# SeanNaren/deepspeech.pytorch

Measured on AMD Instinct MI355X. Metric: audio-seconds/sec (train step), higher is better.
Workload: dtype bf16

## Files before the change

deepspeech/pytorch_amd/_lib.py:

```python
import ctypes as C
import os

HERE = os.path.dirname(os.path.abspath(__file__))
LIB_PATH = os.path.join(HERE, "libds2hip.so")

F32, BF16 = 0, 1
CELL_GRU, CELL_LSTM, CELL_RNN_TANH = 0, 1, 2

_vp, _i, _l, _f, _ll = C.c_void_p, C.c_int, C.c_long, C.c_float, C.c_longlong

SIGNATURES = {
    "ds2_version": (_i, []),
    "ds2_error_string": (C.c_char_p, [_i]),
    "ds2_gemm_nt": (_i, [_i, _vp, _vp, _vp, _vp, _i, _i, _i, _l, _l, _l, _i, _i, _l, _l, _l, _l, _i, _vp]),
    "ds2_gemm_nt_coresident": (_i, [_i, _vp, _vp, _vp, _vp, _i, _i, _i, _l, _l, _l, _i, _i, _l, _l, _l, _l, _i, _vp]),
    "ds2_gemm_nt_rows2": (_i, [_i, _vp, _vp, _i, _vp, _vp, _i, _i, _i, _l, _l, _l, _i, _i, _i, _vp]),
    "ds2_gemm8_nt": (_i, [_vp, _vp, _vp, _vp, _i, _i, _i, _l, _l, _l, _i, _vp]),
    "ds2_gemm8_tn_grouped": (_i, [_i, _vp, _vp, _vp, _vp, _vp, _vp, _vp, _vp, _vp, _vp, _vp, _i, _vp]),
    "ds2_gemm8_nt_rows": (_i, [_vp, _vp, _vp, _vp, _i, _i, _i, _l, _l, _l, _i, _vp, _i, _vp]),
    "ds2_gemm8_tn_grouped_rows": (_i, [_i, _vp, _vp, _vp, _vp, _vp, _vp, _vp, _vp, _vp, _vp, _vp, _i, _vp, _i, _vp]),
    "ds2_gemm8_wgrad_dx_rows": (_i, [_i, _vp, _vp, _vp, _vp, _vp, _vp, _vp, _vp, _vp, _vp, _vp, _i, _vp, _vp, _vp, _i, _i, _i, _l, _l, _l, _vp, _i, _vp]),
    "ds2_zero_pad_rows": (_i, [_i, _vp, _l, _i, _vp, _i, _i, _vp]),
    "ds2_gemm8_wgrad_dx": (_i, [_i, _vp, _vp, _vp, _vp, _vp, _vp, _vp, _vp, _vp, _vp, _vp, _i, _vp, _vp, _vp, _i, _i, _i, _l, _l, _l, _vp]),
    "ds2_norm_partials": (_i, [_l]),
    "ds2_bn_fwd": (_i, [_i, _i, _i, _vp, _vp, _l, _i, _l, _l, _i, _i, _i, _vp, _vp, _vp, _vp, _vp, _vp, _f, _f, _vp, _vp,
                        _vp, _vp, _vp, _vp]),
    "ds2_bn_bwd": (_i, [_i, _i, _vp, _vp, _vp, _l, _i, _l, _l, _l, _i, _i, _i, _vp, _vp, _vp, _vp, _vp, _vp, _vp, _vp, _vp]),
    "ds2_colsum": (_i, [_i, _vp, _l, _i, _l, _vp, _f, _vp, _vp]),
    "ds2_conv_rows": (_i, [_i, _vp, _vp]),
    "ds2_conv1_fwd": (_i, [_i, _vp, _vp, _vp, _vp, _vp, _i, _i, _i, _i, _vp]),
    "ds2_conv1_wgrad_ws_floats": (_l, [_i, _i, _i]),
    "ds2_conv1_wgrad": (_i, [_i, _vp, _vp, _vp, _i, _i, _i, _i, _vp, _vp]),
    "ds2_conv2_fwd_ws_bytes": (_l, [_i, _i, _i, _i]),
    "ds2_conv2_fwd": (_i, [_i, _vp, _vp, _vp, _vp, _vp, _i, _i, _i, _vp, _vp]),
    "ds2_conv2_dgrad": (_i, [_i, _vp, _vp, _vp, _vp, _i, _i, _i, _vp]),
    "ds2_conv2_wgrad_ws_floats": (_l, [_i, _i]),
    "ds2_conv2_wgrad": (_i, [_i, _vp, _vp, _vp, _i, _i, _i, _vp, _vp]),
    "ds2_rnn_gates": (_i, [_i]),
    "ds2_rnn_saved_planes": (_i, [_i]),
    "ds2_rnn_state_bytes": (_l, [_i, _i, _i]),
    "ds2_rnn_fwd": (_i, [_i, _i, _i, _i, _i, _i, _vp, _vp, _vp, _vp, _vp, _vp, _vp, _l, _vp, _vp, _vp, _vp, _vp]),
    "ds2_rnn_bwd": (_i, [_i, _i, _i, _i, _i, _i, _vp, _vp, _vp, _vp, _l, _vp, _vp, _vp, _vp, _vp, _vp, _vp, _vp, _vp]),
    "ds2_rnn_persist_plan": (_i, [_i, _i, _i, _i, _i, _i, C.c_uint, C.POINTER(_l)]),
    "ds2_rnn_persist_supported": (_i, [_i, _i, _i, _i, _i, C.c_uint]),
    "ds2_rnn_persist_shape_covered": (_i, [_i, _i, _i, _i, _i]),
    "ds2_rnn_persist_kind": (_i, [_i, _i, _i, _i, _i, C.c_uint]),
    "ds2_rnn_persist_ws_bytes": (_l, [_i, _i, _i, _i, _i, C.c_uint]),
    "ds2_rnn_persist_fwd": (_i, [_i, _i, _i, _i, _i, _i, _vp, _vp, _vp, _vp, _vp, _vp, _vp, _l, _vp, _vp, _vp, _vp, _vp, _vp, _vp]),
    "ds2_rnn_persist_bwd": (_i, [_i, _i, _i, _i, _i, _i, _vp, _vp, _vp, _vp, _l, _vp, _vp, _vp, _vp, _i, _vp, _vp, _vp, _vp]),
    "ds2_add2": (_i, [_i, _vp, _vp, _vp, _l, _vp]),
    "ds2_sum_slices": (_i, [_vp, _vp, _l, _i, _vp]),
    "ds2_transpose": (_i, [_i, _vp, _vp, _l, _i, _l, _l, _vp]),
    "ds2_split3_bf16": (_i, [_vp, _l, _l, _i, _i, _i, _vp, _l, _vp]),
    "ds2_cast_transpose_bf16": (_i, [_vp, _l, _i, _i, _i, _i, _i, _vp, _l, _vp, _l, _vp]),
    "ds2_small_weight_layouts": (_i, [_i, _vp, _vp, _vp, _i, _i, _vp, _vp, _vp, _vp, _vp, _vp, _vp]),
    "ds2_scale_by": (_i, [_vp, _vp, _l, _vp]),
    "ds2_copy_words": (_i, [_vp, _vp, _l, _vp]),
    "ds2_lookahead_fwd": (_i, [_i, _vp, _vp, _vp, _vp, _i, _i, _i, _i, _vp]),
# ... 97 lines not shown
```

deepspeech/pytorch_amd/csrc/ds2_conv.hip:

```cpp
#include "ds2_common.h"

namespace {

constexpr int F0 = 161, F1 = 81, F2 = 41, CH = 32;
constexpr int K1F = 41, K1T = 11, K2F = 21, K2T = 11;

constexpr int C1_FB = 4, C1_TB = 64;
constexpr int C1_PR = (C1_FB - 1) * 2 + K1F;
constexpr int C1_PC = (C1_TB - 1) * 2 + K1T;
constexpr int C1_PCP = C1_PC + 1;

__device__ __forceinline__ void conv1_load_patch(float* patch, const float* __restrict__ xn, int T, int f_base, int t_base,
                                                 int tid, int nthreads, int f0) {
  for (int i = tid; i < C1_PR * C1_PC; i += nthreads) {
    const int pr = i / C1_PC, pc = i - pr * C1_PC;
    const int fi = f_base + pr, ti = t_base + pc;
    const bool ok = fi >= 0 && fi < f0 && ti >= 0 && ti < T;
    const float v = xn[(long)min(max(fi, 0), f0 - 1) * T + min(max(ti, 0), T - 1)];
    patch[pr * C1_PCP + pc] = ok ? v : 0.f;
  }
}

template <typename T>
__global__ void __launch_bounds__(256) k_conv1_fwd(const float* __restrict__ x, const float* __restrict__ w1k,
// ... 557 lines not shown
                                          const CwdNext& nx) {
  constexpr int c = KS & 1, n = c ^ 1, DYB = cwd_dy_bytes(KSN);
  CWD_WAIT_LGKM0();
  __builtin_amdgcn_sched_barrier(0);
#define CWD_SLOT(M)                                                                          \
  Mma<bf16_t>::mma32(acc[(M) / 3][(M) % 3], cwd_frag(fa[c][(M) / 3]), cwd_frag(fb[c][(M) % 3])); \
  if constexpr (KS + 1 < KSN) {                                                              \
    CWD_READ(fa[n], fb[n], KS + 1, 2 * (M));                                                 \
    CWD_READ(fa[n], fb[n], KS + 1, 2 * (M) + 1);                                             \
  }                                                                                          \
  if constexpr ((M) == 8) cwd_dma_dy<KSN, KS>(nx);                                           \
  if constexpr ((M) == 10 && KS < 3) cwd_dma_x<KSN, KS>(nx);                                 \
  __builtin_amdgcn_sched_barrier(0);
  CWD_SLOT(0) CWD_SLOT(1) CWD_SLOT(2) CWD_SLOT(3) CWD_SLOT(4) CWD_SLOT(5)
  CWD_SLOT(6) CWD_SLOT(7) CWD_SLOT(8) CWD_SLOT(9) CWD_SLOT(10) CWD_SLOT(11)
#undef CWD_SLOT
}

constexpr int CWD_UNITS_PER_XCD = 64;
static_assert(CWR_SPLITS * 6 <= 8 * CWD_UNITS_PER_XCD, "every (split, row group) needs a workgroup slot");

template <int KSN>
__global__ void __launch_bounds__(256, cwd_wgs_per_cu(KSN)) k_conv2_wgrad_bf16d(const bf16_t* __restrict__ dY, const bf16_t* __restrict__ A1,
                                                                                float* __restrict__ partial, int N, int Tp, int nsplit) {
  constexpr int R = 4;
  constexpr int TB = 16 * KSN, DYB = cwd_dy_bytes(KSN), BUF = cwd_buf_bytes(KSN);
  static_assert(KSN >= 3 && KSN <= 8, "X chunks: at most three per wave; DMA pieces: one dY chunk per k-step");
  const int unit = (blockIdx.x & 7) * CWD_UNITS_PER_XCD + (blockIdx.x >> 3);
  if (unit >= nsplit * 6) return;
  const int split = unit / 6, rg = unit - split * 6;
  const int kf0 = rg < 3 ? 8 * rg : 1 + 8 * (rg - 3);
  extern __shared__ __attribute__((aligned(16))) unsigned char cwd_smem[];
  const int tid = threadIdx.x, lane = tid & 63, wave = __builtin_amdgcn_readfirstlane(tid >> 6);
  const int li = lane & 31;
  ds2_f32x16 acc[R][3];
#pragma unroll
  for (int r = 0; r < R; ++r)
#pragma unroll
    for (int i = 0; i < 3; ++i)
#pragma unroll
      for (int e = 0; e < 16; ++e) acc[r][i][e] = 0.f;
  const int ntiles = (Tp + TB - 1) / TB;
  constexpr int NJ = F2 + R - 1;
  struct Cursor {
    int n, j, t;
  };
  const int d_t = nsplit % ntiles, d_q = nsplit / ntiles, d_j = d_q % NJ, d_n = d_q / NJ;
  auto advance = [&](Cursor& c) {
    c.t += d_t;
    if (c.t >= ntiles) { c.t -= ntiles; c.j += 1; }
    c.j += d_j;
    if (c.j >= NJ) { c.j -= NJ; c.n += 1; }
    c.n += d_n;
  };
  auto next_live = [&](Cursor c) {
    for (; c.n < N; advance(c)) {
      const int fi = 2 * c.j - 10 + kf0;
      if (fi >= 0 && fi < F1) break;
    }
    return c;
  };
  const int row_bytes = Tp * CH * 2;
  const __amdgpu_buffer_rsrc_t rdy = __builtin_amdgcn_make_buffer_rsrc((void*)dY, 0, N * F2 * row_bytes, 0x00020000);
  const __amdgpu_buffer_rsrc_t rx = __builtin_amdgcn_make_buffer_rsrc((void*)A1, 0, N * F1 * row_bytes, 0x00020000);
  const int lpos = lane >> 2, lbyte = (lane & 3) * 16;
  auto plan = [&](const Cursor& c, int b) {
    CwdNext nx;
    nx.rdy = rdy;
    nx.rx = rx;
    nx.base = cwd_smem + b * BUF;
    nx.Tp = Tp;
    nx.wave = wave;
    nx.lpos = lpos;
    nx.lbyte = lbyte;
    nx.any = c.n < N;
    const int n = nx.any ? c.n : 0;
    const int fi = min(max(2 * c.j - 10 + kf0, 0), F1 - 1);
    const int fo = c.j - wave;
    nx.row_ok = nx.any && fo >= 0 && fo < F2 && kf0 + 2 * wave < K2F;
    nx.soff = __builtin_amdgcn_readfirstlane(nx.row_ok ? (n * F2 + fo) * row_bytes : 0);
    nx.sxoff = __builtin_amdgcn_readfirstlane((n * F1 + fi) * row_bytes);
// ... 55 lines not shown
#pragma unroll
    for (int i = 0; i < 3; ++i) {
      const int kt = wave + 4 * i;
      if (kt < K2T && kf0 + 2 * r < K2F) {
        float* out = partial + (((long)split * K2F + (kf0 + 2 * r)) * K2T + kt) * (CH * CH);
#pragma unroll
        for (int e = 0; e < 16; ++e) out[mma32_row(e, lane) * 32 + li] = acc[r][i][e];
      }
    }
}

struct RTapArgs {
  const bf16_t* X;
  const bf16_t* W;
  const float* bias;
  const int* lens;
  const float* Pin;
  float* Pout;
  bf16_t* Y;
  int N, Tp, Fin, Fout;
  int KF, WSF, WQ;
  int ISF, IQ, PF;
  int U, OSF, OQ;
};
constexpr int RT_FB = 4, RT_TB = 32, RT_PC = RT_TB + K2T - 1;
constexpr int RT_KFM = 11, RT_PR = RT_FB - 1 + RT_KFM;
constexpr int RT_PCD = 48, RT_ROWB = RT_PCD * CH * 2;
constexpr int RT_PATCH = RT_PR * RT_ROWB;
constexpr int RT_RED = 4 * RT_FB * 4096;
constexpr int RT_SMEM = 2 * RT_PATCH + RT_RED;
#define RT_RD128(dst, addr, off) asm volatile("ds_read_b128 %0, %1 offset:%2" : "=v"(dst) : "v"(addr), "i"(off))

struct RtNext {
  __amdgpu_buffer_rsrc_t rx;
  unsigned char* patch;
  int n, ub, tb;
  int Fin, Tp, PF, ISF, IQ;
  int wave, lane;
};
template <int PR, int I>
__device__ __forceinline__ void rt_dma_piece(const RtNext& nx) {
  constexpr int k = I % 3;
  const int pr = nx.wave + 4 * (I / 3);
  if (pr < PR) {
    const int fi = (nx.ub * RT_FB + pr - nx.PF) * nx.ISF + nx.IQ;
    const bool row_ok = nx.n >= 0 && fi >= 0 && fi < nx.Fin;
    const int soff = __builtin_amdgcn_readfirstlane(row_ok ? (nx.n * nx.Fin + fi) * (nx.Tp * CH * 2) : 0);
    const int pc = 16 * k + (nx.lane >> 2), ti = nx.tb * RT_TB - 5 + pc;
    const int voff = (row_ok && pc < RT_PC && (unsigned)ti < (unsigned)nx.Tp) ? ti * (CH * 2) + (((nx.lane & 3) ^ (nx.lane >> 4)) << 4) : CW_OOB;
    __builtin_amdgcn_raw_ptr_buffer_load_lds(nx.rx, (cw_lds_ptr_t)(nx.patch + pr * RT_ROWB + k * 1024), 16, voff, soff, 0, 0);
  }
}
template <int PR, int I>
__device__ __forceinline__ void rt_dma_all(const RtNext& nx) {
  rt_dma_piece<PR, I>(nx);
  if constexpr (I + 1 < 12) rt_dma_all<PR, I + 1>(nx);
}
constexpr int RT_AH = 4;
template <int ST>
__device__ __forceinline__ void rt_prefetch(uint4 (&bq)[RT_AH + 1], const uint32_t (&aj)[6]) {
  RT_RD128(bq[ST], aj[ST % 6], (ST / 6) * RT_ROWB);
  if constexpr (ST + 1 < RT_AH) rt_prefetch<ST + 1>(bq, aj);
}
template <int KF, int ST>
__device__ __forceinline__ void rt_step(ds2_f32x16 (&acc)[RT_FB], const uint4 (&A)[KF][6], uint4 (&bq)[RT_AH + 1], const uint32_t (&aj)[6],
                                        const RtNext& nx) {
  constexpr int PR = RT_FB - 1 + KF, NS = PR * 6, rho = ST / 6, j = ST % 6;
  if constexpr (ST + RT_AH < NS) RT_RD128(bq[(ST + RT_AH) % (RT_AH + 1)], aj[(ST + RT_AH) % 6], ((ST + RT_AH) / 6) * RT_ROWB);
  constexpr int left = RT_AH < NS - 1 - ST ? RT_AH : NS - 1 - ST;
  if constexpr (left >= 4) asm volatile("s_waitcnt lgkmcnt(4)" ::: "memory");
  else if constexpr (left == 3) asm volatile("s_waitcnt lgkmcnt(3)" ::: "memory");
  else if constexpr (left == 2) asm volatile("s_waitcnt lgkmcnt(2)" ::: "memory");
  else if constexpr (left == 1) asm volatile("s_waitcnt lgkmcnt(1)" ::: "memory");
  else asm volatile("s_waitcnt lgkmcnt(0)" ::: "memory");
  __builtin_amdgcn_sched_barrier(0);
#pragma unroll
  for (int fl = 0; fl < RT_FB; ++fl) {
    const int m = rho - fl;
    if (m >= 0 && m < KF) Mma<bf16_t>::mma32(acc[fl], A[m][j], bq[ST % (RT_AH + 1)]);
  }
  if constexpr (ST % 6 == 3 && ST >= 9 && (ST - 9) / 6 < 12) rt_dma_piece<PR, (ST - 9) / 6>(nx);
  __builtin_amdgcn_sched_barrier(0);
  if constexpr (ST + 1 < NS) rt_step<KF, ST + 1>(acc, A, bq, aj, nx);
}

template <int KF>
__global__ void __launch_bounds__(256, 1) k_conv_rtap(RTapArgs a) {
  extern __shared__ __attribute__((aligned(16))) unsigned char rsm[];
  float* red = reinterpret_cast<float*>(rsm + 2 * RT_PATCH);
  const int tid = threadIdx.x, lane = tid & 63, wave = __builtin_amdgcn_readfirstlane(tid >> 6);
  const int li = lane & 31, lq = lane >> 5;
  const int i0 = wave < 2 ? 6 * wave : 12 + 5 * (wave - 2), icnt = wave < 2 ? 6 : 5;
  uint4 A[KF][6];
  const uint32_t lds0 = (uint32_t)(uintptr_t)(__attribute__((address_space(3))) unsigned char*)rsm;
  uint32_t boff[6];
#pragma unroll
  for (int j = 0; j < 6; ++j) {
    const int item = i0 + min(j, icnt - 1), kt = item >> 1, half = item & 1;
    const int p = li + kt;
    boff[j] = lds0 + p * (CH * 2) + (((half * 2 + lq) ^ ((p >> 2) & 3)) << 4);
#pragma unroll
    for (int m = 0; m < KF; ++m) {
      const uint4 wv = *reinterpret_cast<const uint4*>(a.W + (((long)(m * a.WSF + a.WQ) * K2T + kt) * CH + li) * CH + half * 16 + lq * 8);
      A[m][j] = j < icnt ? wv : make_uint4(0u, 0u, 0u, 0u);
    }
  }
#ifndef DS2_RTAP_VKEEP
#define DS2_RTAP_VKEEP 24
#endif
#pragma unroll
  for (int m = 0; m < KF; ++m)
#pragma unroll
    for (int j = 0; j < 6; ++j)
      if (m * 6 + j >= DS2_RTAP_VKEEP) {
        typedef __attribute__((ext_vector_type(4))) unsigned int u4v;
        u4v v = __builtin_bit_cast(u4v, A[m][j]);
        asm volatile("" : "+a"(v));
        A[m][j] = __builtin_bit_cast(uint4, v);
      }
  constexpr int PR = RT_FB - 1 + KF;
  constexpr int NPIECE = 12;
  const int nub = ds2_cdiv_dev(a.U, RT_FB), ntb = ds2_cdiv_dev(a.Tp, RT_TB);
  const int total = a.N * nub * ntb;
  RtNext nx;
  nx.rx = __builtin_amdgcn_make_buffer_rsrc((void*)a.X, 0, a.N * a.Fin * a.Tp * CH * 2, 0x00020000);
  nx.Fin = a.Fin; nx.Tp = a.Tp; nx.PF = a.PF; nx.ISF = a.ISF; nx.IQ = a.IQ;
  nx.wave = wave; nx.lane = lane;
  auto aim = [&](int tile, int buf) {
    const bool any = tile < total;
    const int tt = any ? tile : 0;
    nx.tb = tt % ntb;
    nx.ub = (tt / ntb) % nub;
    nx.n = any ? tt / (ntb * nub) : -1;
    nx.patch = rsm + buf * RT_PATCH;
  };

  int tile = blockIdx.x;
  if (tile < total) {
    aim(tile, 0);
    rt_dma_all<PR, 0>(nx);
  }
  __syncthreads();
  int buf = 0;
  for (; tile < total; tile += gridDim.x, buf ^= 1) {
    const int tb = tile % ntb, ub = (tile / ntb) % nub, n = tile / (ntb * nub);
    const int next = tile + gridDim.x;
    aim(next, buf ^ 1);
    float4 pin[4];
    {
      const int u = ub * RT_FB + wave, t = tb * RT_TB + li;
      const bool have = a.Pin != nullptr && u < a.U && t < a.Tp;
      const float* src = a.Pin + (((long)n * a.U + min(u, a.U - 1)) * a.Tp + min(t, a.Tp - 1)) * CH + 4 * lq;
#pragma unroll
      for (int g = 0; g < 4; ++g) pin[g] = have ? *reinterpret_cast<const float4*>(src + 8 * g) : make_float4(0.f, 0.f, 0.f, 0.f);
    }
    ds2_f32x16 acc[RT_FB];
#pragma unroll
    for (int fl = 0; fl < RT_FB; ++fl)
#pragma unroll
      for (int r = 0; r < 16; ++r) acc[fl][r] = 0.f;
    {
      uint4 bq[RT_AH + 1];
      uint32_t aj[6];
#pragma unroll
      for (int j = 0; j < 6; ++j) aj[j] = boff[j] + buf * RT_PATCH;
      __builtin_amdgcn_sched_barrier(0);
      rt_prefetch<0>(bq, aj);
      rt_step<KF, 0>(acc, A, bq, aj, nx);
    }
#pragma unroll
    for (int fl = 0; fl < RT_FB; ++fl)
#pragma unroll
      for (int g = 0; g < 4; ++g)
        *reinterpret_cast<float4*>(red + (((wave * RT_FB + fl) * 4 + g) * 64 + lane) * 4) =
            make_float4(acc[fl][4 * g], acc[fl][4 * g + 1], acc[fl][4 * g + 2], acc[fl][4 * g + 3]);
    asm volatile("s_waitcnt vmcnt(0)" ::: "memory");
    __syncthreads();
    {
      const int u = ub * RT_FB + wave, t = tb * RT_TB + li;
      float o[16];
#pragma unroll
      for (int g = 0; g < 4; ++g) {
        float4 s4 = *reinterpret_cast<const float4*>(red + (((0 * RT_FB + wave) * 4 + g) * 64 + lane) * 4);
#pragma unroll
        for (int w = 1; w < 4; ++w) {
          const float4 q4 = *reinterpret_cast<const float4*>(red + (((w * RT_FB + wave) * 4 + g) * 64 + lane) * 4);
          s4.x += q4.x; s4.y += q4.y; s4.z += q4.z; s4.w += q4.w;
        }
        o[4 * g] = s4.x; o[4 * g + 1] = s4.y; o[4 * g + 2] = s4.z; o[4 * g + 3] = s4.w;
      }
      if (u < a.U && t < a.Tp) {
        const long pidx = (((long)n * a.U + u) * a.Tp + t) * CH + 4 * lq;
        if (a.Pin) {
#pragma unroll
          for (int g = 0; g < 4; ++g) {
            o[4 * g] += pin[g].x; o[4 * g + 1] += pin[g].y; o[4 * g + 2] += pin[g].z; o[4 * g + 3] += pin[g].w;
          }
        }
// ... 132 lines not shown
    static bool attr[DS2_MAX_DEVICES];
    if (ds2_first_use_on_device(attr))
      (void)hipFuncSetAttribute((const void*)k_conv1_wgrad_mfma, hipFuncAttributeMaxDynamicSharedMemorySize, M1W_SMEM);
    P = conv1_wgrad_mfma_blocks(N, Tp) < P ? conv1_wgrad_mfma_blocks(N, Tp) : P;
    hipLaunchKernelGGL(k_conv1_wgrad_mfma, dim3(P), dim3(256), M1W_SMEM, st, x, (const bf16_t*)dy1, ws, N, T, Tp, ds2_cdiv(Tp, M1_TB));
  }
  DS2_CHECK_LAUNCH();
  const int C = K1F * K1T * CH;
  return ds2_colsum(DS2_F32, ws, P, C, C, dw1k, 1.0f, ws + (long)P * C, st_);
}

long ds2_conv2_fwd_ws_bytes(int dtype, int N, int F0_, int Tp) { return (dtype == DS2_BF16 && F0_ == F0) ? (long)N * F2 * Tp * CH * 4 : 0; }
int ds2_conv2_fwd(int dtype, const void* a1, const void* w2t, const float* b2, const int* lens, void* y2, int N, int F0_, int Tp, void* ws,
                  ds2_stream_t st_) {
  hipStream_t st = (hipStream_t)st_;
  DS2_REQUIRE(dtype == DS2_F32 || dtype == DS2_BF16, DS2_ERR_DTYPE);
  int f1, f2;
  DS2_REQUIRE(N > 0 && Tp > 0 && conv_geometry(F0_, f1, f2), DS2_ERR_ARG);
  if (dtype == DS2_F32 || F0_ != F0 || (long)N * F1 * Tp * CH * 2 >= (long)CW_OOB) {
    ConvTapArgs a{a1, w2t, b2, lens, y2, N, Tp, f1, f2, K2F, 2, 10, f2, 1, 0};
    return dtype == DS2_F32 ? conv_tap_launch<float>(a, st) : conv_tap_launch<bf16_t>(a, st);
  }
  DS2_REQUIRE(ws != nullptr, DS2_ERR_ARG);
  RTapArgs e{(const bf16_t*)a1, (const bf16_t*)w2t, nullptr, nullptr, nullptr, (float*)ws, nullptr, N, Tp, F1, F2, 11, 2, 0, 2, 0, 5, F2, 1, 0};
  RTapArgs o{(const bf16_t*)a1, (const bf16_t*)w2t, b2, lens, (const float*)ws, nullptr, (bf16_t*)y2, N, Tp, F1, F2, 10, 2, 1, 2, 1, 5, F2, 1, 0};
  const int rc = conv_rtap_launch(e, st);
  return rc ? rc : conv_rtap_launch(o, st);
}

int ds2_conv2_dgrad(int dtype, const void* dy2, const void* w2d_even, const void* w2d_odd, void* da1, int N, int F0_, int Tp,
                    ds2_stream_t st_) {
  hipStream_t st = (hipStream_t)st_;
  DS2_REQUIRE(dtype == DS2_F32 || dtype == DS2_BF16, DS2_ERR_DTYPE);
  int f1, f2;
  DS2_REQUIRE(N > 0 && Tp > 0 && conv_geometry(F0_, f1, f2), DS2_ERR_ARG);
  if (dtype == DS2_BF16 && F0_ == F0 && (long)N * F1 * Tp * CH * 2 < (long)CW_OOB) {
    RTapArgs e{(const bf16_t*)dy2, (const bf16_t*)w2d_even, nullptr, nullptr, nullptr, nullptr, (bf16_t*)da1, N, Tp, F2, F1, 11, 1, 0, 1, 0, 5, 41, 2, 0};
    RTapArgs o{(const bf16_t*)dy2, (const bf16_t*)w2d_odd, nullptr, nullptr, nullptr, nullptr, (bf16_t*)da1, N, Tp, F2, F1, 10, 1, 0, 1, 0, 4, 40, 2, 1};
    const int rc = conv_rtap_launch(e, st);
    return rc ? rc : conv_rtap_launch(o, st);
  }
  ConvTapArgs e{dy2, w2d_even, nullptr, nullptr, da1, N, Tp, f2, f1, 11, 1, 5, (f1 + 1) / 2, 2, 0};
  ConvTapArgs o{dy2, w2d_odd, nullptr, nullptr, da1, N, Tp, f2, f1, 10, 1, 4, f1 / 2, 2, 1};
  if (dtype == DS2_F32) {
    const int rc = conv_tap_launch<float>(e, st);
    return (rc || f1 / 2 == 0) ? rc : conv_tap_launch<float>(o, st);
  }
  const int rc = conv_tap_launch<bf16_t>(e, st);
  return (rc || f1 / 2 == 0) ? rc : conv_tap_launch<bf16_t>(o, st);
}

long ds2_conv2_wgrad_ws_floats(int N, int Tp) {
  (void)N; (void)Tp;
  const long C = (long)K2F * K2T * CH * CH;
  static_assert(CWR_SPLITS >= CW_SPLITS, "sized for the larger split count of the two kernels");
  return (long)CWR_SPLITS * C + (long)ds2_norm_partials(CWR_SPLITS) * C;
}
int ds2_conv2_wgrad(int dtype, const void* dy2, const void* a1, float* dw2t, int N, int F0_, int Tp, float* ws, ds2_stream_t st_) {
  hipStream_t st = (hipStream_t)st_;
  DS2_REQUIRE(dtype == DS2_F32 || dtype == DS2_BF16, DS2_ERR_DTYPE);
  int f1, f2;
  DS2_REQUIRE(conv_geometry(F0_, f1, f2), DS2_ERR_ARG);
  dim3 grid(K2F, CW_SPLITS);
  const bool general = dtype == DS2_F32 || F0_ != F0 || (long)N * F1 * Tp * CH * 2 >= (long)CW_OOB;
  if (dtype == DS2_F32) {
    hipLaunchKernelGGL(k_conv2_wgrad<float>, grid, dim3(256), 0, st, (const float*)dy2, (const float*)a1, ws, N, Tp, f1, f2);
  } else if (general) {
    hipLaunchKernelGGL(k_conv2_wgrad<bf16_t>, grid, dim3(256), 0, st, (const bf16_t*)dy2, (const bf16_t*)a1, ws, N, Tp, f1, f2);
  } else {
    static bool attr[DS2_MAX_DEVICES];
    constexpr int smem = cwd_smem_bytes(CWD_KSN);
    if (ds2_first_use_on_device(attr))
      (void)hipFuncSetAttribute((const void*)k_conv2_wgrad_bf16d<CWD_KSN>, hipFuncAttributeMaxDynamicSharedMemorySize, smem);
    hipLaunchKernelGGL(k_conv2_wgrad_bf16d<CWD_KSN>, dim3(8 * CWD_UNITS_PER_XCD), dim3(256), smem, st, (const bf16_t*)dy2, (const bf16_t*)a1, ws, N,
                       Tp, CWR_SPLITS);
  }
  DS2_CHECK_LAUNCH();
  const int C = K2F * K2T * CH * CH;
  const int splits = general ? CW_SPLITS : CWR_SPLITS;
  return ds2_colsum(DS2_F32, ws, splits, C, C, dw2t, 1.0f, ws + (long)splits * C, st_);
}

}
```

deepspeech/pytorch_amd/model.py:

```python
import math
from typing import List

import numpy as np
import torch
import torch.nn as nn

from . import ops
from ._lib import Ds2HipError

try:
    import pytorch_lightning as pl
    _Base = pl.LightningModule
except Exception:
    pl = None

    class _Base(nn.Module):

        def save_hyperparameters(self, *a, **k):
            import inspect
            frame = inspect.currentframe().f_back
            try:
                names = [n for n in inspect.signature(type(self).__init__).parameters if n != "self"]
                self._hparams = {n: frame.f_locals[n] for n in names if n in frame.f_locals}
            finally:
# ... 53 lines not shown
        dirs = (2, 1) if bidirectional is None else ((2,) if bidirectional else (1,))
        for w in range(base, int(base * 1.5) + 1, 16):
            if any(query("ds2_rnn_persist_shape_covered", dt_, cell, D_, 1, w) for D_ in dirs):
                return w
    except Exception:
        pass
    return base


def _data_parallel_active():
    if PER_LAYER_NODES_FOR_DDP[0]:
        return True
    try:
        import torch.distributed as _dist
        return _dist.is_available() and _dist.is_initialized() and _dist.get_world_size() > 1
    except Exception:
        return False


FP32_WGRAD_TN = os.environ.get("DS2_FP32_WGRAD_TN", "1") != "0"

ROW_LISTS = os.environ.get("DS2_ROW_LISTS", "1") != "0"
ROW_LIST_MIN_PADDING = 0.97

N_FREQ_CONV2 = 41
RNN_INPUT = 32 * N_FREQ_CONV2
RNN_INPUT_LD = 1344


def _round64(n):
    return (n + 63) // 64 * 64


class SequenceWise(nn.Module):
    def __init__(self, module):
        super().__init__()
        self.module = module


class MaskConv(nn.Module):
    def __init__(self, seq_module):
        super().__init__()
        self.seq_module = seq_module


class _RNNParams(nn.Module):
# ... 147 lines not shown
        x0 = torch.empty((Tp * N, rld), dtype=dtype, device=x.device)
        if rld > rin:
            x0[:, rin:].zero_()
        sv2 = ops.bn_fwd(y2, 2, training, g2.detach(), be2.detach(), bn2.running_mean, bn2.running_var,
                         bn2.num_batches_tracked, R2, 32, 32, x0, rld, F=F2, Tp=Tp, N=N, lens=lens_dev, eps=bn2.eps,
                         momentum=bn2.momentum)
        ctx.mod, ctx.dims, ctx.sv = mod, (N, T, Tp, dtype), (sv1, sv2)
        ctx.save_for_backward(x, y1, a1, y2, lens_dev, w2)
        return x0

    @staticmethod
    def backward(ctx, dx0):
        x, y1, a1, y2, lens_dev, w2 = ctx.saved_tensors
        N, T, Tp, dtype = ctx.dims
        sv1, sv2 = ctx.sv
        c = ctx.mod._cache
        dx0 = dx0.contiguous().to(dtype)
        F0, F1, F2, rld = ctx.mod._F0, ctx.mod._F1, ctx.mod._F2, ctx.mod._rnn_ld
        R1, R2 = N * F1 * Tp, N * F2 * Tp
        dy2 = torch.empty_like(y2)
        dg2, dbe2 = ops.bn_bwd(dx0, y2, dy2, 2, sv2, R2, 32, rld, 32, 32, F=F2, Tp=Tp, N=N, lens=lens_dev)
        w2d = c.get(("w2d", dtype), [w2], lambda: [
            w2.detach()[:, :, q::2, :].flip(2, 3).permute(2, 3, 1, 0).contiguous().to(dtype) for q in (0, 1)])
        da1 = ops.conv2_dgrad(dy2, w2d[0], w2d[1], F0)
        dy1 = torch.empty_like(y1)
        dg1, dbe1 = ops.bn_bwd(da1, y1, dy1, 1, sv1, R1, 32, 32, 32, 32, F=F1, Tp=Tp, N=N, lens=lens_dev)
        db1 = ops.colsum(dy1.view(R1, 32))
        dw1k = ops.conv1_wgrad(x, dy1, Tp)
        dw1 = dw1k.t().reshape(32, 1, 41, 11).contiguous()
        db2 = ops.colsum(dy2.view(R2, 32))
        dw2 = ops.conv2_wgrad(dy2, a1, F0).view(21, 11, 32, 32).permute(2, 3, 0, 1).contiguous()
        return (None, dw1, db1, dg1, dbe1, dw2, db2, dg2, dbe2, None, None, None, None, None)


def _layer_param_count(layer):
    return (2 if layer.batch_norm is not None else 0) + 4 * layer.num_directions


_ROWS_STAGING, _CTC_STAGING = ops.PinnedRing(), ops.PinnedRing()


def _frame_rows(output_lengths, Tp, N, dev):
    ol = output_lengths.numpy().astype(np.int32)
    n_valid = int(np.minimum(ol, Tp).sum())
    if not ROW_LISTS or n_valid >= ROW_LIST_MIN_PADDING * Tp * N or n_valid == 0:
        return output_lengths.to(dev, torch.int32, non_blocking=True), None
    rows = np.flatnonzero(np.arange(Tp, dtype=np.int32)[:, None] < ol[None, :]).astype(np.int32)
    both = _ROWS_STAGING.stage(dev, [ol, rows])
    return both[:N], both[N:]


def _rnn_layer_forward(mod, li, X, lens_dev, N, Tp, dtype, training, h0, c0, lparams, rows=None):
    c = mod._cache
    R = Tp * N
# ... 956 lines not shown
```

deepspeech/pytorch_amd/ops.py:

```python
import ctypes as C

import numpy as np
import torch

from . import _lib
from ._lib import F32, BF16, call, query

CELLS = {"gru": _lib.CELL_GRU, "lstm": _lib.CELL_LSTM, "rnn": _lib.CELL_RNN_TANH}
GATES = {"gru": 3, "lstm": 4, "rnn": 1}
SAVED_PLANES = {"gru": 4, "lstm": 5, "rnn": 0}


def dt(t):
    d = t if isinstance(t, torch.dtype) else t.dtype
    if d == torch.float32:
        return F32
    if d == torch.bfloat16:
        return BF16
    raise TypeError("ds2hip supports float32 and bfloat16 activations, got %s" % d)


def vecw(dtype):
    return 4 if dtype == torch.float32 else 8

# ... 369 lines not shown
    y1 = torch.empty((N, conv_rows(F0)[0], Tp, 32), dtype=dtype, device=x.device)
    call("ds2_conv1_fwd", dt(dtype), PF(x), PF(w1k), PF(b1), P(lens), P(y1), N, F0, T, Tp, S())
    return y1


def conv1_wgrad(x, dy1, Tp):
    N, _, F0, T = x.shape
    dw = torch.empty((451, 32), dtype=torch.float32, device=x.device)
    ws = torch.empty(query("ds2_conv1_wgrad_ws_floats", N, F0, Tp), dtype=torch.float32, device=x.device)
    call("ds2_conv1_wgrad", dt(dy1), P(x), P(dy1), P(dw), N, F0, T, Tp, P(ws), S())
    return dw


def conv2_fwd(a1, w2t, b2, lens, F0=161):
    N, F1, Tp, _ = a1.shape
    assert F1 == conv_rows(F0)[0]
    y2 = torch.empty((N, conv_rows(F0)[1], Tp, 32), dtype=a1.dtype, device=a1.device)
    nws = query("ds2_conv2_fwd_ws_bytes", dt(a1), N, F0, Tp)
    ws = torch.empty(nws, dtype=torch.uint8, device=a1.device) if nws else None
    call("ds2_conv2_fwd", dt(a1), P(a1), P(w2t), PF(b2), P(lens), P(y2), N, F0, Tp, P(ws), S())
    return y2


def conv2_dgrad(dy2, w2d_even, w2d_odd, F0=161):
    N, F2, Tp, _ = dy2.shape
    assert F2 == conv_rows(F0)[1]
    da1 = torch.empty((N, conv_rows(F0)[0], Tp, 32), dtype=dy2.dtype, device=dy2.device)
    call("ds2_conv2_dgrad", dt(dy2), P(dy2), P(w2d_even), P(w2d_odd), P(da1), N, F0, Tp, S())
    return da1


def conv2_wgrad(dy2, a1, F0=161):
    N, _, Tp, _ = dy2.shape
    dw = torch.empty((231, 32, 32), dtype=torch.float32, device=dy2.device)
    ws = torch.empty(query("ds2_conv2_wgrad_ws_floats", N, Tp), dtype=torch.float32, device=dy2.device)
    call("ds2_conv2_wgrad", dt(dy2), P(dy2), P(a1), P(dw), N, F0, Tp, P(ws), S())
    return dw


_PERSIST_ERR = {}
LAST_PERSIST_WS = None

STARTUP_MS_SINGLE = 300
STARTUP_MS_DP_MIN, STARTUP_MS_DP_MAX = 30_000, 3_600_000
_OPTS = {"variant": 0, "spin_limit": 0, "startup_ms": None}
FORCE_DATA_PARALLEL_BUDGET = [False]


class persist_options:

    def __init__(self, **kw):
        assert set(kw) <= set(_OPTS), kw
        self.kw = kw

    def __enter__(self):
        self.old = dict(_OPTS)
        _OPTS.update(self.kw)
        return self

# ... 897 lines not shown
```

include/ds2hip.h:

```cpp
#ifndef DS2HIP_H
#define DS2HIP_H

#include <stdint.h>

#ifdef __cplusplus
extern "C" {
#endif

typedef void* ds2_stream_t;

enum { DS2_F32 = 0, DS2_BF16 = 1 };
enum { DS2_CELL_GRU = 0, DS2_CELL_LSTM = 1, DS2_CELL_RNN_TANH = 2 };
enum {
  DS2_OK = 0,
  DS2_ERR_DTYPE = 1001,
  DS2_ERR_ARG = 1002,
  DS2_ERR_ALIGN = 1003
};

int ds2_version(void);
const char* ds2_error_string(int code);

int ds2_gemm_nt(int dtype, const void* A, const void* B, void* C, const float* bias, int M, int N, int K, long lda, long ldb,
                long ldc, int out_f32, int batch, long strideA, long strideB, long strideC, long strideBias, int splitk,
// ... 30 lines not shown
int ds2_bn_fwd(int dtype, int mode, int training, const void* X, void* Y, long R, int C, long ldx, long ldy, int F, int Tp,
               int N, const int* lens, const float* gamma, const float* beta, float* running_mean, float* running_var,
               long long* num_batches_tracked, float eps, float momentum, float* save_mean, float* save_rstd,
               float* save_scale, float* save_shift, float* ws, ds2_stream_t stream);
int ds2_bn_bwd(int dtype, int mode, const void* G, const void* X, void* DX, long R, int C, long ldg, long ldx, long lddx,
               int F, int Tp, int N, const int* lens, const float* save_mean, const float* save_rstd,
               const float* save_scale, const float* save_shift, float* dgamma, float* dbeta, float* ws,
               ds2_stream_t stream);
int ds2_colsum(int dtype, const void* X, long R, int C, long ld, float* out, float scale, float* ws, ds2_stream_t stream);

int ds2_conv_rows(int F0, int* F1, int* F2);
int ds2_conv1_fwd(int dtype, const float* x, const float* w1k, const float* b1, const int* lens, void* y1, int N, int F0, int T,
                  int Tp, ds2_stream_t stream);
long ds2_conv1_wgrad_ws_floats(int N, int F0, int Tp);
int ds2_conv1_wgrad(int dtype, const float* x, const void* dy1, float* dw1k, int N, int F0, int T, int Tp, float* ws,
                    ds2_stream_t stream);
long ds2_conv2_fwd_ws_bytes(int dtype, int N, int F0, int Tp);
int ds2_conv2_fwd(int dtype, const void* a1, const void* w2t, const float* b2, const int* lens, void* y2, int N, int F0, int Tp,
                  void* ws, ds2_stream_t stream);
int ds2_conv2_dgrad(int dtype, const void* dy2, const void* w2d_even, const void* w2d_odd, void* da1, int N, int F0, int Tp,
                    ds2_stream_t stream);
long ds2_conv2_wgrad_ws_floats(int N, int Tp);
int ds2_conv2_wgrad(int dtype, const void* dy2, const void* a1, float* dw2t, int N, int F0, int Tp, float* ws, ds2_stream_t stream);

int ds2_rnn_gates(int cell);
int ds2_rnn_saved_planes(int cell);
long ds2_rnn_state_bytes(int D, int N, int H);
int ds2_rnn_fwd(int dtype, int cell, int D, int N, int H, int Tp, const int* lens, const void* GI, const void* Whh,
                const float* bhh, const float* h0, const float* c0, void* Hseq, long hseq_dstride, void* S, float* hn, float* cn,
                void* state, ds2_stream_t stream);
int ds2_rnn_bwd(int dtype, int cell, int D, int N, int H, int Tp, const int* lens, const void* dOut, const void* WhhT,
                const void* Hseq, long hseq_dstride, const void* S, void* dGI, void* dGH, const float* h0, const float* c0,
                float* dh0, float* dc0, void* state, ds2_stream_t stream);

typedef struct ds2_persist_opts {
  unsigned variant;
  unsigned spin_limit;
  unsigned startup_ms;
} ds2_persist_opts;
int ds2_rnn_persist_plan(int dtype, int cell, int D, int N, int H, int cus, unsigned variant, long* ws_bytes);
int ds2_rnn_persist_supported(int dtype, int cell, int D, int N, int H, unsigned variant);
int ds2_rnn_persist_shape_covered(int dtype, int cell, int D, int N, int H);
int ds2_rnn_persist_kind(int dtype, int cell, int D, int N, int H, unsigned variant);
long ds2_rnn_persist_ws_bytes(int dtype, int cell, int D, int N, int H, unsigned variant);
int ds2_rnn_persist_fwd(int dtype, int cell, int D, int N, int H, int Tp, const int* lens, const void* GI, const void* Whh,
                        const float* bhh, const float* h0, const float* c0, void* Hseq, long hseq_dstride, void* S, float* hn,
// ... 132 lines not shown
```

Before: 21930.

## Skip padded time tiles in conv2 forward, dgrad and wgrad using sequence lengths

Passes per-utterance lengths into the conv2 register-tap kernels and the wgrad kernel so tiles lying entirely in time padding are not computed. Instead, their outputs are zero-filled directly. Tile indexing becomes a prefix sum over per-sample tile counts, built with a wave scan. A separate single-row multiply variant handles a leftover output-row tail when the row count is not a multiple of the row block. This removes MMA and DMA work on padded frames in variable-length batches, at the cost of more complex scheduling and a sample-count limit of 64 for skipping.

```diff
diff --git a/deepspeech/pytorch_amd/_lib.py b/deepspeech/pytorch_amd/_lib.py
--- a/deepspeech/pytorch_amd/_lib.py
+++ b/deepspeech/pytorch_amd/_lib.py
@@ -34,6 +34,8 @@
     "ds2_conv2_fwd_ws_bytes": (_l, [_i, _i, _i, _i]),
     "ds2_conv2_fwd": (_i, [_i, _vp, _vp, _vp, _vp, _vp, _i, _i, _i, _vp, _vp]),
     "ds2_conv2_dgrad": (_i, [_i, _vp, _vp, _vp, _vp, _i, _i, _i, _vp]),
+    "ds2_conv2_dgrad_lens": (_i, [_i, _vp, _vp, _vp, _vp, _vp, _i, _i, _i, _vp]),
+    "ds2_conv2_wgrad_lens": (_i, [_i, _vp, _vp, _vp, _vp, _i, _i, _i, _vp, _vp]),
     "ds2_conv2_wgrad_ws_floats": (_l, [_i, _i]),
     "ds2_conv2_wgrad": (_i, [_i, _vp, _vp, _vp, _i, _i, _i, _vp, _vp]),
     "ds2_rnn_gates": (_i, [_i]),
diff --git a/deepspeech/pytorch_amd/csrc/ds2_conv.hip b/deepspeech/pytorch_amd/csrc/ds2_conv.hip
--- a/deepspeech/pytorch_amd/csrc/ds2_conv.hip
+++ b/deepspeech/pytorch_amd/csrc/ds2_conv.hip
@@ -1,4 +1,6 @@
 #include "ds2_common.h"
+
+#include <type_traits>
 
 namespace {
 
@@ -603,7 +605,8 @@
 
 template <int KSN>
 __global__ void __launch_bounds__(256, cwd_wgs_per_cu(KSN)) k_conv2_wgrad_bf16d(const bf16_t* __restrict__ dY, const bf16_t* __restrict__ A1,
-                                                                                float* __restrict__ partial, int N, int Tp, int nsplit) {
+                                                                                float* __restrict__ partial, int N, int Tp, int nsplit,
+                                                                                const int* __restrict__ lens) {
   constexpr int R = 4;
   constexpr int TB = 16 * KSN, DYB = cwd_dy_bytes(KSN), BUF = cwd_buf_bytes(KSN);
   static_assert(KSN >= 3 && KSN <= 8, "X chunks: at most three per wave; DMA pieces: one dY chunk per k-step");
@@ -637,7 +640,7 @@
   auto next_live = [&](Cursor c) {
     for (; c.n < N; advance(c)) {
       const int fi = 2 * c.j - 10 + kf0;
-      if (fi >= 0 && fi < F1) break;
+      if (fi >= 0 && fi < F1 && (lens == nullptr || c.t * TB < lens[c.n])) break;
     }
     return c;
   };
@@ -739,7 +742,12 @@
   int KF, WSF, WQ;
   int ISF, IQ, PF;
   int U, OSF, OQ;
+  const int* skip_lens;
 };
+#ifndef DS2_RTAP_TAIL
+#define DS2_RTAP_TAIL 1
+#endif
+constexpr int RT_SKIP_NMAX = 64;
 constexpr int RT_FB = 4, RT_TB = 32, RT_PC = RT_TB + K2T - 1;
 constexpr int RT_KFM = 11, RT_PR = RT_FB - 1 + RT_KFM;
 constexpr int RT_PCD = 48, RT_ROWB = RT_PCD * CH * 2;
@@ -779,10 +787,12 @@
   RT_RD128(bq[ST], aj[ST % 6], (ST / 6) * RT_ROWB);
   if constexpr (ST + 1 < RT_AH) rt_prefetch<ST + 1>(bq, aj);
 }
-template <int KF, int ST>
-__device__ __forceinline__ void rt_step(ds2_f32x16 (&acc)[RT_FB], const uint4 (&A)[KF][6], uint4 (&bq)[RT_AH + 1], const uint32_t (&aj)[6],
+template <int KF, int FB, int ST>
+__device__ __forceinline__ void rt_step(ds2_f32x16 (&acc)[FB], const uint4 (&A)[KF][6], uint4 (&bq)[RT_AH + 1], const uint32_t (&aj)[6],
                                         const RtNext& nx) {
-  constexpr int PR = RT_FB - 1 + KF, NS = PR * 6, rho = ST / 6, j = ST % 6;
+  constexpr int PR = FB - 1 + KF, NS = PR * 6, rho = ST / 6, j = ST % 6;
+  constexpr int NP = 3 * ((PR + 3) / 4);
+  static_assert(FB == 1 || (NS - 3 - 9) / 6 + 1 >= NP, "every DMA piece of the next patch has a step to ride on");
   if constexpr (ST + RT_AH < NS) RT_RD128(bq[(ST + RT_AH) % (RT_AH + 1)], aj[(ST + RT_AH) % 6], ((ST + RT_AH) / 6) * RT_ROWB);
   constexpr int left = RT_AH < NS - 1 - ST ? RT_AH : NS - 1 - ST;
   if constexpr (left >= 4) asm volatile("s_waitcnt lgkmcnt(4)" ::: "memory");
@@ -792,13 +802,17 @@
   else asm volatile("s_waitcnt lgkmcnt(0)" ::: "memory");
   __builtin_amdgcn_sched_barrier(0);
 #pragma unroll
-  for (int fl = 0; fl < RT_FB; ++fl) {
+  for (int fl = 0; fl < FB; ++fl) {
     const int m = rho - fl;
     if (m >= 0 && m < KF) Mma<bf16_t>::mma32(acc[fl], A[m][j], bq[ST % (RT_AH + 1)]);
   }
-  if constexpr (ST % 6 == 3 && ST >= 9 && (ST - 9) / 6 < 12) rt_dma_piece<PR, (ST - 9) / 6>(nx);
+  if constexpr (FB == 1) {
+    if constexpr (ST < NP) rt_dma_piece<PR, ST>(nx);
+  } else if constexpr (ST % 6 == 3 && ST >= 9 && (ST - 9) / 6 < 12) {
+    rt_dma_piece<PR, (ST - 9) / 6>(nx);
+  }
   __builtin_amdgcn_sched_barrier(0);
-  if constexpr (ST + 1 < NS) rt_step<KF, ST + 1>(acc, A, bq, aj, nx);
+  if constexpr (ST + 1 < NS) rt_step<KF, FB, ST + 1>(acc, A, bq, aj, nx);
 }
 
 template <int KF>
@@ -838,31 +852,103 @@
   constexpr int PR = RT_FB - 1 + KF;
   constexpr int NPIECE = 12;
   const int nub = ds2_cdiv_dev(a.U, RT_FB), ntb = ds2_cdiv_dev(a.Tp, RT_TB);
-  const int total = a.N * nub * ntb;
+  const bool skip = a.skip_lens != nullptr && a.N <= RT_SKIP_NMAX;
+  int inc = 0;
+  if (skip) {
+    if (lane < a.N) inc = (min(max(a.skip_lens[lane], 0), a.Tp) + RT_TB - 1) / RT_TB;
+#pragma unroll
+    for (int d = 1; d < 64; d <<= 1) {
+      const int up = __shfl_up(inc, d, 64);
+      if (lane >= d) inc += up;
+    }
+  }
+  auto pre = [&](int n) { return skip ? (n > 0 ? __builtin_amdgcn_readlane(inc, n - 1) : 0) : n * ntb; };
+  const bool has_tail = DS2_RTAP_TAIL && a.U % RT_FB == 1;
+  const int nfull = has_tail ? nub - 1 : nub;
+  const int E1 = nfull * pre(a.N), E2 = E1 + (has_tail ? pre(a.N) : 0);
+  struct Tile {
+    int idx, n, ub, tb;
+    bool tail;
+  };
+  auto seek = [&](Tile& c, int idx) {
+    c.idx = idx;
+    if (idx >= E2) {
+      c.n = -1;
+      c.ub = c.tb = 0;
+    } else if (idx < E1) {
+      int n = c.n;
+      while (idx >= nfull * pre(n + 1)) ++n;
+      const int p = pre(n), r = idx - nfull * p, ln = pre(n + 1) - p;
+      c.n = n;
+      c.ub = r / ln;
+      c.tb = r - c.ub * ln;
+    } else {
+      int n = c.tail ? c.n : 0;
+      const int j = idx - E1;
+      while (j >= pre(n + 1)) ++n;
+      c.n = n;
+      c.ub = nub - 1;
+      c.tb = j - pre(n);
+      c.tail = true;
+    }
+    c.n = __builtin_amdgcn_readfirstlane(c.n); c.ub = __builtin_amdgcn_readfirstlane(c.ub); c.tb = __builtin_amdgcn_readfirstlane(c.tb);
+  };
+  if (skip && a.Pout == nullptr) {
+    const int rows = a.N * a.U;
+    for (int r = blockIdx.x; r < rows; r += gridDim.x) {
+      const int n = r / a.U, u = r - n * a.U;
+      const int t0 = min((pre(n + 1) - pre(n)) * RT_TB, a.Tp);
+      uint4* dst = reinterpret_cast<uint4*>(a.Y + (((long)n * a.Fout + u * a.OSF + a.OQ) * a.Tp + t0) * CH);
+      for (int c = tid; c < (a.Tp - t0) * (CH * 2 / 16); c += 256) dst[c] = make_uint4(0u, 0u, 0u, 0u);
+    }
+  }
   RtNext nx;
   nx.rx = __builtin_amdgcn_make_buffer_rsrc((void*)a.X, 0, a.N * a.Fin * a.Tp * CH * 2, 0x00020000);
   nx.Fin = a.Fin; nx.Tp = a.Tp; nx.PF = a.PF; nx.ISF = a.ISF; nx.IQ = a.IQ;
   nx.wave = wave; nx.lane = lane;
-  auto aim = [&](int tile, int buf) {
-    const bool any = tile < total;
-    const int tt = any ? tile : 0;
-    nx.tb = tt % ntb;
-    nx.ub = (tt / ntb) % nub;
-    nx.n = any ? tt / (ntb * nub) : -1;
+  auto aim = [&](const Tile& t, int buf) {
+    nx.tb = t.tb;
+    nx.ub = t.ub;
+    nx.n = t.n;
     nx.patch = rsm + buf * RT_PATCH;
   };
-
-  int tile = blockIdx.x;
-  if (tile < total) {
-    aim(tile, 0);
+  auto multiply = [&](auto fbc, int buf) {
+    constexpr int FB = decltype(fbc)::value;
+    ds2_f32x16 acc[FB];
+#pragma unroll
+    for (int fl = 0; fl < FB; ++fl)
+#pragma unroll
+      for (int r = 0; r < 16; ++r) acc[fl][r] = 0.f;
+    {
+      uint4 bq[RT_AH + 1];
+      uint32_t aj[6];
+#pragma unroll
+      for (int j = 0; j < 6; ++j) aj[j] = boff[j] + buf * RT_PATCH;
+      __builtin_amdgcn_sched_barrier(0);
+      rt_prefetch<0>(bq, aj);
+      rt_step<KF, FB, 0>(acc, A, bq, aj, nx);
+    }
+#pragma unroll
+    for (int fl = 0; fl < FB; ++fl)
+#pragma unroll
+      for (int g = 0; g < 4; ++g)
+        *reinterpret_cast<float4*>(red + (((wave * RT_FB + fl) * 4 + g) * 64 + lane) * 4) =
+            make_float4(acc[fl][4 * g], acc[fl][4 * g + 1], acc[fl][4 * g + 2], acc[fl][4 * g + 3]);
+  };
+
+  Tile cur{0, 0, 0, 0, false};
+  seek(cur, blockIdx.x);
+  Tile nxt = cur;
+  if (cur.n >= 0) {
+    seek(nxt, cur.idx + gridDim.x);
+    aim(cur, 0);
     rt_dma_all<PR, 0>(nx);
   }
   __syncthreads();
   int buf = 0;
-  for (; tile < total; tile += gridDim.x, buf ^= 1) {
-    const int tb = tile % ntb, ub = (tile / ntb) % nub, n = tile / (ntb * nub);
-    const int next = tile + gridDim.x;
-    aim(next, buf ^ 1);
+  for (; cur.n >= 0; buf ^= 1) {
+    const int tb = cur.tb, ub = cur.ub, n = cur.n;
+    aim(nxt, buf ^ 1);
     float4 pin[4];
     {
       const int u = ub * RT_FB + wave, t = tb * RT_TB + li;
@@ -871,26 +957,10 @@
 #pragma unroll
       for (int g = 0; g < 4; ++g) pin[g] = have ? *reinterpret_cast<const float4*>(src + 8 * g) : make_float4(0.f, 0.f, 0.f, 0.f);
     }
-    ds2_f32x16 acc[RT_FB];
-#pragma unroll
-    for (int fl = 0; fl < RT_FB; ++fl)
-#pragma unroll
-      for (int r = 0; r < 16; ++r) acc[fl][r] = 0.f;
-    {
-      uint4 bq[RT_AH + 1];
-      uint32_t aj[6];
-#pragma unroll
-      for (int j = 0; j < 6; ++j) aj[j] = boff[j] + buf * RT_PATCH;
-      __builtin_amdgcn_sched_barrier(0);
-      rt_prefetch<0>(bq, aj);
-      rt_step<KF, 0>(acc, A, bq, aj, nx);
-    }
-#pragma unroll
-    for (int fl = 0; fl < RT_FB; ++fl)
-#pragma unroll
-      for (int g = 0; g < 4; ++g)
-        *reinterpret_cast<float4*>(red + (((wave * RT_FB + fl) * 4 + g) * 64 + lane) * 4) =
-            make_float4(acc[fl][4 * g], acc[fl][4 * g + 1], acc[fl][4 * g + 2], acc[fl][4 * g + 3]);
+    if (cur.tail) multiply(std::integral_constant<int, 1>{}, buf);
+    else multiply(std::integral_constant<int, RT_FB>{}, buf);
+    cur = nxt;
+    if (nxt.n >= 0) seek(nxt, nxt.idx + gridDim.x);
     asm volatile("s_waitcnt vmcnt(0)" ::: "memory");
     __syncthreads();
     {
@@ -1069,21 +1139,23 @@
     return dtype == DS2_F32 ? conv_tap_launch<float>(a, st) : conv_tap_launch<bf16_t>(a, st);
   }
   DS2_REQUIRE(ws != nullptr, DS2_ERR_ARG);
-  RTapArgs e{(const bf16_t*)a1, (const bf16_t*)w2t, nullptr, nullptr, nullptr, (float*)ws, nullptr, N, Tp, F1, F2, 11, 2, 0, 2, 0, 5, F2, 1, 0};
-  RTapArgs o{(const bf16_t*)a1, (const bf16_t*)w2t, b2, lens, (const float*)ws, nullptr, (bf16_t*)y2, N, Tp, F1, F2, 10, 2, 1, 2, 1, 5, F2, 1, 0};
+  const int* skip = N <= RT_SKIP_NMAX ? lens : nullptr;
+  RTapArgs e{(const bf16_t*)a1, (const bf16_t*)w2t, nullptr, nullptr, nullptr, (float*)ws, nullptr, N, Tp, F1, F2, 11, 2, 0, 2, 0, 5, F2, 1, 0, skip};
+  RTapArgs o{(const bf16_t*)a1, (const bf16_t*)w2t, b2, lens, (const float*)ws, nullptr, (bf16_t*)y2, N, Tp, F1, F2, 10, 2, 1, 2, 1, 5, F2, 1, 0, skip};
   const int rc = conv_rtap_launch(e, st);
   return rc ? rc : conv_rtap_launch(o, st);
 }
 
-int ds2_conv2_dgrad(int dtype, const void* dy2, const void* w2d_even, const void* w2d_odd, void* da1, int N, int F0_, int Tp,
-                    ds2_stream_t st_) {
+int ds2_conv2_dgrad_lens(int dtype, const void* dy2, const void* w2d_even, const void* w2d_odd, const int* lens, void* da1, int N,
+                         int F0_, int Tp, ds2_stream_t st_) {
   hipStream_t st = (hipStream_t)st_;
   DS2_REQUIRE(dtype == DS2_F32 || dtype == DS2_BF16, DS2_ERR_DTYPE);
   int f1, f2;
   DS2_REQUIRE(N > 0 && Tp > 0 && conv_geometry(F0_, f1, f2), DS2_ERR_ARG);
   if (dtype == DS2_BF16 && F0_ == F0 && (long)N * F1 * Tp * CH * 2 < (long)CW_OOB) {
-    RTapArgs e{(const bf16_t*)dy2, (const bf16_t*)w2d_even, nullptr, nullptr, nullptr, nullptr, (bf16_t*)da1, N, Tp, F2, F1, 11, 1, 0, 1, 0, 5, 41, 2, 0};
-    RTapArgs o{(const bf16_t*)dy2, (const bf16_t*)w2d_odd, nullptr, nullptr, nullptr, nullptr, (bf16_t*)da1, N, Tp, F2, F1, 10, 1, 0, 1, 0, 4, 40, 2, 1};
+    const int* skip = N <= RT_SKIP_NMAX ? lens : nullptr;
+    RTapArgs e{(const bf16_t*)dy2, (const bf16_t*)w2d_even, nullptr, nullptr, nullptr, nullptr, (bf16_t*)da1, N, Tp, F2, F1, 11, 1, 0, 1, 0, 5, 41, 2, 0, skip};
+    RTapArgs o{(const bf16_t*)dy2, (const bf16_t*)w2d_odd, nullptr, nullptr, nullptr, nullptr, (bf16_t*)da1, N, Tp, F2, F1, 10, 1, 0, 1, 0, 4, 40, 2, 1, skip};
     const int rc = conv_rtap_launch(e, st);
     return rc ? rc : conv_rtap_launch(o, st);
   }
@@ -1096,6 +1168,10 @@
   const int rc = conv_tap_launch<bf16_t>(e, st);
   return (rc || f1 / 2 == 0) ? rc : conv_tap_launch<bf16_t>(o, st);
 }
+int ds2_conv2_dgrad(int dtype, const void* dy2, const void* w2d_even, const void* w2d_odd, void* da1, int N, int F0_, int Tp,
+                    ds2_stream_t st_) {
+  return ds2_conv2_dgrad_lens(dtype, dy2, w2d_even, w2d_odd, nullptr, da1, N, F0_, Tp, st_);
+}
 
 long ds2_conv2_wgrad_ws_floats(int N, int Tp) {
   (void)N; (void)Tp;
@@ -1103,7 +1179,8 @@
   static_assert(CWR_SPLITS >= CW_SPLITS, "sized for the larger split count of the two kernels");
   return (long)CWR_SPLITS * C + (long)ds2_norm_partials(CWR_SPLITS) * C;
 }
-int ds2_conv2_wgrad(int dtype, const void* dy2, const void* a1, float* dw2t, int N, int F0_, int Tp, float* ws, ds2_stream_t st_) {
+int ds2_conv2_wgrad_lens(int dtype, const void* dy2, const void* a1, const int* lens, float* dw2t, int N, int F0_, int Tp, float* ws,
+                         ds2_stream_t st_) {
   hipStream_t st = (hipStream_t)st_;
   DS2_REQUIRE(dtype == DS2_F32 || dtype == DS2_BF16, DS2_ERR_DTYPE);
   int f1, f2;
@@ -1120,12 +1197,15 @@
     if (ds2_first_use_on_device(attr))
       (void)hipFuncSetAttribute((const void*)k_conv2_wgrad_bf16d<CWD_KSN>, hipFuncAttributeMaxDynamicSharedMemorySize, smem);
     hipLaunchKernelGGL(k_conv2_wgrad_bf16d<CWD_KSN>, dim3(8 * CWD_UNITS_PER_XCD), dim3(256), smem, st, (const bf16_t*)dy2, (const bf16_t*)a1, ws, N,
-                       Tp, CWR_SPLITS);
+                       Tp, CWR_SPLITS, lens);
   }
   DS2_CHECK_LAUNCH();
   const int C = K2F * K2T * CH * CH;
   const int splits = general ? CW_SPLITS : CWR_SPLITS;
   return ds2_colsum(DS2_F32, ws, splits, C, C, dw2t, 1.0f, ws + (long)splits * C, st_);
 }
-
-}
+int ds2_conv2_wgrad(int dtype, const void* dy2, const void* a1, float* dw2t, int N, int F0_, int Tp, float* ws, ds2_stream_t st_) {
+  return ds2_conv2_wgrad_lens(dtype, dy2, a1, nullptr, dw2t, N, F0_, Tp, ws, st_);
+}
+
+}
diff --git a/deepspeech/pytorch_amd/model.py b/deepspeech/pytorch_amd/model.py
--- a/deepspeech/pytorch_amd/model.py
+++ b/deepspeech/pytorch_amd/model.py
@@ -99,6 +99,7 @@
 
 ROW_LISTS = os.environ.get("DS2_ROW_LISTS", "1") != "0"
 ROW_LIST_MIN_PADDING = 0.97
+CONV_SKIP_PADDING = os.environ.get("DS2_CONV_SKIP_PADDING", "1") != "0"
 
 N_FREQ_CONV2 = 41
 RNN_INPUT = 32 * N_FREQ_CONV2
@@ -292,14 +293,15 @@
         dg2, dbe2 = ops.bn_bwd(dx0, y2, dy2, 2, sv2, R2, 32, rld, 32, 32, F=F2, Tp=Tp, N=N, lens=lens_dev)
         w2d = c.get(("w2d", dtype), [w2], lambda: [
             w2.detach()[:, :, q::2, :].flip(2, 3).permute(2, 3, 1, 0).contiguous().to(dtype) for q in (0, 1)])
-        da1 = ops.conv2_dgrad(dy2, w2d[0], w2d[1], F0)
+        skip_lens = lens_dev if CONV_SKIP_PADDING else None
+        da1 = ops.conv2_dgrad(dy2, w2d[0], w2d[1], F0, lens=skip_lens)
         dy1 = torch.empty_like(y1)
         dg1, dbe1 = ops.bn_bwd(da1, y1, dy1, 1, sv1, R1, 32, 32, 32, 32, F=F1, Tp=Tp, N=N, lens=lens_dev)
         db1 = ops.colsum(dy1.view(R1, 32))
         dw1k = ops.conv1_wgrad(x, dy1, Tp)
         dw1 = dw1k.t().reshape(32, 1, 41, 11).contiguous()
         db2 = ops.colsum(dy2.view(R2, 32))
-        dw2 = ops.conv2_wgrad(dy2, a1, F0).view(21, 11, 32, 32).permute(2, 3, 0, 1).contiguous()
+        dw2 = ops.conv2_wgrad(dy2, a1, F0, lens=skip_lens).view(21, 11, 32, 32).permute(2, 3, 0, 1).contiguous()
         return (None, dw1, db1, dg1, dbe1, dw2, db2, dg2, dbe2, None, None, None, None, None)
 
 
diff --git a/deepspeech/pytorch_amd/ops.py b/deepspeech/pytorch_amd/ops.py
--- a/deepspeech/pytorch_amd/ops.py
+++ b/deepspeech/pytorch_amd/ops.py
@@ -415,19 +415,25 @@
     return y2
 
 
-def conv2_dgrad(dy2, w2d_even, w2d_odd, F0=161):
+def conv2_dgrad(dy2, w2d_even, w2d_odd, F0=161, lens=None):
     N, F2, Tp, _ = dy2.shape
     assert F2 == conv_rows(F0)[1]
     da1 = torch.empty((N, conv_rows(F0)[0], Tp, 32), dtype=dy2.dtype, device=dy2.device)
-    call("ds2_conv2_dgrad", dt(dy2), P(dy2), P(w2d_even), P(w2d_odd), P(da1), N, F0, Tp, S())
+    if lens is None:
+        call("ds2_conv2_dgrad", dt(dy2), P(dy2), P(w2d_even), P(w2d_odd), P(da1), N, F0, Tp, S())
+    else:
+        call("ds2_conv2_dgrad_lens", dt(dy2), P(dy2), P(w2d_even), P(w2d_odd), P(lens), P(da1), N, F0, Tp, S())
     return da1
 
 
-def conv2_wgrad(dy2, a1, F0=161):
+def conv2_wgrad(dy2, a1, F0=161, lens=None):
     N, _, Tp, _ = dy2.shape
     dw = torch.empty((231, 32, 32), dtype=torch.float32, device=dy2.device)
     ws = torch.empty(query("ds2_conv2_wgrad_ws_floats", N, Tp), dtype=torch.float32, device=dy2.device)
-    call("ds2_conv2_wgrad", dt(dy2), P(dy2), P(a1), P(dw), N, F0, Tp, P(ws), S())
+    if lens is None:
+        call("ds2_conv2_wgrad", dt(dy2), P(dy2), P(a1), P(dw), N, F0, Tp, P(ws), S())
+    else:
+        call("ds2_conv2_wgrad_lens", dt(dy2), P(dy2), P(a1), P(lens), P(dw), N, F0, Tp, P(ws), S())
     return dw
 
 
diff --git a/include/ds2hip.h b/include/ds2hip.h
--- a/include/ds2hip.h
+++ b/include/ds2hip.h
@@ -76,6 +76,10 @@
                     ds2_stream_t stream);
 long ds2_conv2_wgrad_ws_floats(int N, int Tp);
 int ds2_conv2_wgrad(int dtype, const void* dy2, const void* a1, float* dw2t, int N, int F0, int Tp, float* ws, ds2_stream_t stream);
+int ds2_conv2_dgrad_lens(int dtype, const void* dy2, const void* w2d_even, const void* w2d_odd, const int* lens, void* da1, int N,
+                         int F0, int Tp, ds2_stream_t stream);
+int ds2_conv2_wgrad_lens(int dtype, const void* dy2, const void* a1, const int* lens, float* dw2t, int N, int F0, int Tp, float* ws,
+                         ds2_stream_t stream);
 
 int ds2_rnn_gates(int cell);
 int ds2_rnn_saved_planes(int cell);
```

Result: no change. 22030 (median of 6 runs) (+0.4%).
